# moonbow721/DPoser

Measured on AMD Instinct MI355X. Metric: poses/sec score-net train step (subVP DSM, ScoreModelFC) at global B=65536, higher is better.
Workload: dtype bf16; 1 GPU; subVP denoising-score-matching train step (fwd+bwd+clip+Adam+EMA), ScoreModelFC H=1024 E=512 2 blocks, z-scored toy-pose rows [B,63]; global_batch=65536, per_gpu_batch=65536, parallelism=dp1

## Files before the change

dposer_amd/csrc/elementwise.hip:

```cpp
#include "kernels_api.h"
#include "sde_dev.h"
#include "rng.h"

#pragma clang fp contract(off)


template <typename T> __device__ __forceinline__ void store_quad_ft(void* base, int64_t s, int c, int K, f32x4 v) {
    Quad<T>::store(reinterpret_cast<T*>(base) + FT<T>::index(s, c, K), v);
}

template <bool FAST = false>
__device__ __forceinline__ float temb_from_freq(float label, bool sin_half, float f, int fourier) {
    float arg;
    if (fourier) arg = ((logf(label) * f) * 2.0f) * 3.14159274101257324f;
    else arg = label * f;
    if (FAST && !fourier) {
        const float rev = arg * 0.15915494309189535f;
        return sin_half ? __builtin_amdgcn_sinf(rev) : __builtin_amdgcn_cosf(rev);
    }
    return sin_half ? sinf(arg) : cosf(arg);
}
template <bool FAST = false>
__device__ __forceinline__ float temb_value(float label, int e, int E, const float* freq, int fourier) {
    const int half = E >> 1;
    return temb_from_freq<FAST>(label, e < half, freq[e < half ? e : e - half], fourier);
}

template <typename Job> __device__ __forceinline__ Job kernarg_job(int index) {
    static_assert(sizeof(Job) % 4 == 0, "jobs are copied as dwords");
    typedef const uint32_t __attribute__((address_space(4))) * ConstWords;
    ConstWords w = (ConstWords)__builtin_amdgcn_kernarg_segment_ptr() + (size_t)index * (sizeof(Job) / 4);
    union { Job j; uint32_t u[sizeof(Job) / 4]; } c;
#pragma unroll
    for (unsigned i = 0; i < sizeof(Job) / 4; ++i) c.u[i] = w[i];
    return c.j;
}

template <typename T> __device__ __forceinline__ void pack_chunk(const PackJob& j, const float* flat, unsigned char* packed, int64_t chunk) {
    constexpr int EPL = FT<T>::EPL, KBS = FT<T>::KBS;
    const int kblocks = j.kpad / KBS;
    const int lane = (int)(chunk & 63);
    const int64_t blk = chunk >> 6;
    const int kb = (int)(blk % kblocks);
    const int64_t rb = blk / kblocks;
    const int r = (int)(rb * 32 + (lane & 31));
    const int k0 = kb * KBS + (lane >> 5) * EPL;
    const float* src = flat + j.src_off;
    T vals[EPL];
#pragma unroll
    for (int e = 0; e < EPL; ++e) {
        const int k = k0 + e;
        float v = 0.f;
        if (r < j.rows_valid && k < j.cols_valid) v = j.trans ? src[(int64_t)k * j.ld + r] : src[(int64_t)r * j.ld + k];
        if (sizeof(T) == 2 && j.split == 2) v = v - (float)(__bf16)v;
        vals[e] = from_f32<T>(v);
    }
    T* dst = reinterpret_cast<T*>(packed + j.dst_off) + FT<T>::index(r, j.koff + k0, j.ktot);
    *reinterpret_cast<u32x4*>(dst) = *reinterpret_cast<u32x4*>(vals);
}
__global__ void __launch_bounds__(256) k_pack(PackJobs jobs, const float* flat, unsigned char* packed) {
    (void)jobs;
    const PackJob j = kernarg_job<PackJob>((int)blockIdx.y);
    const int epl = j.f32 ? 4 : 8;
    const int64_t nchunks = (int64_t)j.rows_pad * j.kpad / epl;
    for (int64_t c = (int64_t)blockIdx.x * blockDim.x + threadIdx.x; c < nchunks; c += (int64_t)gridDim.x * blockDim.x) {
        if (j.f32) pack_chunk<float>(j, flat, packed, c);
        else pack_chunk<__bf16>(j, flat, packed, c);
    }
}
hipError_t launch_pack(const PackJobs& jobs, const float* flat, void* packed, hipStream_t st) {
    if (jobs.n <= 0) return hipSuccess;
    hipLaunchKernelGGL(k_pack, dim3(256, jobs.n), dim3(256), 0, st, jobs, flat, reinterpret_cast<unsigned char*>(packed));
    return hipGetLastError();
}

__global__ void k_bias_cat(BiasCatJobs j, const float* flat, float* dst) {
    const int i = blockIdx.x * blockDim.x + threadIdx.x;
    if (i >= j.n * j.H) return;
    const int l = i / j.H, c = i % j.H;
    int64_t a = j.a_off[0], b = j.b_off[0];
#pragma unroll
    for (int k = 1; k < 8; ++k) { a = (l == k) ? j.a_off[k] : a; b = (l == k) ? j.b_off[k] : b; }
    dst[i] = flat[a + c] + flat[b + c];
}
hipError_t launch_bias_cat(const BiasCatJobs& j, const float* flat, float* dst, hipStream_t st) {
    const int n = j.n * j.H;
    hipLaunchKernelGGL(k_bias_cat, dim3((n + 255) / 256), dim3(256), 0, st, j, flat, dst);
    return hipGetLastError();
}

template <typename T> __global__ void __launch_bounds__(256) k_prep_infer(PrepArgs a) {
    const int qx = a.Dpad >> 2, qe = a.emb ? (a.E >> 2) : 0;
    const int64_t nx = a.Bpad * qx;
    const int64_t total = nx + a.Bpad * qe;
    for (int64_t i = (int64_t)blockIdx.x * blockDim.x + threadIdx.x; i < total; i += (int64_t)gridDim.x * blockDim.x) {
        const int64_t s = i < nx ? i / qx : (i - nx) % a.Bpad;
        const int q = i < nx ? (int)(i % qx) : qx + (int)((i - nx) / a.Bpad);
        f32x4 v = {0.f, 0.f, 0.f, 0.f};
        if (q < qx) {
            const int c = q * 4;
            if (s < a.B) {
#pragma unroll
                for (int r = 0; r < 4; ++r)
                    if (c + r < a.D) v[r] = a.x[s * a.D + c + r];
            }
            store_quad_ft<T>(a.xin, s, c, a.Dpad, v);
        } else {
            const int e = (q - qx) * 4;
            const float label = s < a.B ? a.labels[s] : (a.fourier ? 1.0f : 0.0f);
#pragma unroll
            for (int r = 0; r < 4; ++r) v[r] = temb_value<sizeof(T) == 2>(label, e + r, a.E, a.freq, a.fourier);
            store_quad_ft<T>(a.emb, s, e, a.E, v);
        }
    }
}
static inline int grid_for(int64_t n, int per_block = 256, int cap = 8192) {
    int64_t g = (n + per_block - 1) / per_block;
    return (int)(g < 1 ? 1 : (g > cap ? cap : g));
}
hipError_t launch_prep_infer(const PrepArgs& a, hipStream_t st) {
    const int64_t total = a.Bpad * ((a.Dpad >> 2) + (a.emb ? (a.E >> 2) : 0));
    if (a.f32) hipLaunchKernelGGL(k_prep_infer<float>, dim3(grid_for(total)), dim3(256), 0, st, a);
    else hipLaunchKernelGGL(k_prep_infer<__bf16>, dim3(grid_for(total)), dim3(256), 0, st, a);
    return hipGetLastError();
}

struct PrepTrainDev {
    PrepTrainArgs a;
    SdeDev sde;
    float t_scale;
};
constexpr int PREP_EQ = 8;
template <typename T, bool FOURIER> __global__ void __launch_bounds__(256) k_prep_train(PrepTrainDev d) {
    const PrepTrainArgs& a = d.a;
    const int qx = a.Dpad >> 2, qe = a.E >> 2;
    const int ge = (qe + PREP_EQ - 1) / PREP_EQ;
    const int QD = (a.D + 3) >> 2;
    const int64_t nx = a.Bpad * qx;
    const int64_t total = nx + a.Bpad * ge;
    for (int64_t i = (int64_t)blockIdx.x * blockDim.x + threadIdx.x; i < total; i += (int64_t)gridDim.x * blockDim.x) {
        const int64_t s = i < nx ? i / qx : (i - nx) % a.Bpad;
        float t = a.eps;
        if (s < a.B) {
            if (a.t_in) t = a.t_in[s];
            else {
                Philox4 r = philox_at((uint64_t)s, STREAM_TRAIN_T, a.step, a.seed);
                t = u01(r.v[0]) * d.t_scale + a.eps;
            }
        }
        if (i < nx) {
            const int q = (int)(i % qx);
            f32x4 v = {0.f, 0.f, 0.f, 0.f};
            const int c = q * 4;
            f32x4 z = {0.f, 0.f, 0.f, 0.f};
            if (s < a.B && c < a.D) {
                if (a.z_in) {
#pragma unroll
                    for (int r = 0; r < 4; ++r)
                        if (c + r < a.D) z[r] = a.z_in[s * a.D + c + r];
                } else {
                    float n4[4];
                    normals4((uint64_t)s * QD + q, STREAM_TRAIN_Z, a.step, a.seed, n4);
#pragma unroll
                    for (int r = 0; r < 4; ++r)
                        if (c + r < a.D) z[r] = n4[r];
                }
                const SdeAt at = sde_at(d.sde, t);
                const float mc = at.mc, sd = at.sd;
#pragma unroll
                for (int r = 0; r < 4; ++r)
                    if (c + r < a.D) v[r] = mc * a.x0[s * a.D + c + r] + sd * z[r];
            }
            store_quad_ft<T>(a.xin, s, c, a.Dpad, v);
            *reinterpret_cast<f32x4*>(a.z_out + s * a.Dpad + c) = z;
            if (q == 0) a.t_out[s] = t;
        } else {
            const int g0 = (int)((i - nx) / a.Bpad) * PREP_EQ;
            const float label = d.sde.kind == SDE_VE ? sde_ve_sigma(d.sde.smin, d.sde.ratio, t) : t * 999.0f;
            const int half = a.E >> 1;
            f32x4 fr[PREP_EQ];
#pragma unroll
            for (int k = 0; k < PREP_EQ; ++k) {
                const int e = (g0 + k) * 4;
                fr[k] = f32x4{0.f, 0.f, 0.f, 0.f};
                if (e < a.E) fr[k] = *reinterpret_cast<const f32x4*>(a.freq + (e < half ? e : e - half));
            }
#pragma unroll
            for (int k = 0; k < PREP_EQ; ++k) {
                const int e = (g0 + k) * 4;
                if (e < a.E) {
                    f32x4 v;
#pragma unroll
                    for (int r = 0; r < 4; ++r) v[r] = temb_from_freq<sizeof(T) == 2>(label, e < half, fr[k][r], FOURIER);
                    store_quad_ft<T>(a.emb, s, e, a.E, v);
                }
            }
        }
    }
}
hipError_t launch_prep_train(const PrepTrainArgs& a, hipStream_t st) {
    PrepTrainDev d;
    d.a = a;
    d.sde = make_sde_dev(a.sde);
    d.t_scale = (float)((double)a.sde.T - (double)a.eps);
    const int64_t total = a.Bpad * ((a.Dpad >> 2) + ((a.E >> 2) + PREP_EQ - 1) / PREP_EQ);
    if (a.fourier) {
        if (a.f32) hipLaunchKernelGGL((k_prep_train<float, true>), dim3(grid_for(total)), dim3(256), 0, st, d);
        else hipLaunchKernelGGL((k_prep_train<__bf16, true>), dim3(grid_for(total)), dim3(256), 0, st, d);
    } else {
        if (a.f32) hipLaunchKernelGGL((k_prep_train<float, false>), dim3(grid_for(total)), dim3(256), 0, st, d);
        else hipLaunchKernelGGL((k_prep_train<__bf16, false>), dim3(grid_for(total)), dim3(256), 0, st, d);
    }
    return hipGetLastError();
}

__global__ void __launch_bounds__(256) k_time_embed(const float* labels, float label0, int64_t n, int64_t npad, const float* freq, int E, int fourier, float* emb) {
    const int qe = E >> 2;
    const int64_t total = npad * qe;
    for (int64_t i = (int64_t)blockIdx.x * blockDim.x + threadIdx.x; i < total; i += (int64_t)gridDim.x * blockDim.x) {
        const int64_t s = i % npad;
        const int e = (int)(i / npad) * 4;
        const float label = s < n ? (labels ? labels[s] : label0) : (fourier ? 1.0f : 0.0f);
        f32x4 v;
#pragma unroll
        for (int r = 0; r < 4; ++r) v[r] = temb_value(label, e + r, E, freq, fourier);
        store_quad_ft<float>(emb, s, e, E, v);
    }
}
__global__ void __launch_bounds__(256) k_ve_labels(float* t_inout, int n, float smin, float ratio) {
    const int i = blockIdx.x * 256 + threadIdx.x;
    if (i < n) t_inout[i] = sde_ve_sigma(smin, ratio, t_inout[i]);
}
hipError_t launch_ve_labels(float* t_inout, int n, float smin, float ratio, hipStream_t st) {
    if (n <= 0) return hipSuccess;
    hipLaunchKernelGGL(k_ve_labels, dim3((unsigned)((n + 255) / 256)), dim3(256), 0, st, t_inout, n, smin, ratio);
    return hipGetLastError();
}
hipError_t launch_time_embed(const float* labels, float label0, int64_t n, int64_t npad, const float* freq, int E, int fourier, float* emb, hipStream_t st) {
    hipLaunchKernelGGL(k_time_embed, dim3(grid_for(npad * (E >> 2))), dim3(256), 0, st, labels, label0, n, npad, freq, E, fourier, emb);
    return hipGetLastError();
}


__global__ void __launch_bounds__(256) k_out_model(OutModelArgs a) {
    const int64_t total = a.B * a.D;
    for (int64_t i = (int64_t)blockIdx.x * blockDim.x + threadIdx.x; i < total; i += (int64_t)gridDim.x * blockDim.x) {
        const int64_t s = i / a.D;
        const int c = (int)(i % a.D);
        float v = a.res[s * a.Cp + c];
        if (a.scale_by_sigma) v = v / used_sigma(a.sigmas, a.num_scales, a.labels[s], a.fourier);
        a.out[i] = v;
    }
}
hipError_t launch_out_model(const OutModelArgs& a, hipStream_t st) {
    hipLaunchKernelGGL(k_out_model, dim3(grid_for(a.B * a.D)), dim3(256), 0, st, a);
    return hipGetLastError();
}

template <typename A> struct WithSde {
    A a;
    SdeDev sde;
};
template <typename A> static hipError_t launch_quads(void (*k32)(WithSde<A>), void (*k16)(WithSde<A>), const A& a, const SdeDev& sde, hipStream_t st) {
    const WithSde<A> d = {a, sde};
    hipLaunchKernelGGL(a.f32 ? k32 : k16, dim3(grid_for(a.Bpad * (a.Dpad >> 2))), dim3(256), 0, st, d);
    return hipGetLastError();
}
template <typename A> __device__ __forceinline__ float launch_usig(const A& a, float label) {
    return a.scale_by_sigma ? used_sigma(a.sigmas, a.num_scales, label, a.scale_by_sigma == 2) : 1.0f;
}
__device__ __forceinline__ float score_of_res(const SdeDev& sde, float res, float usig, float sd_score) { return sde_score(sde, res / usig, sd_score); }
__device__ __forceinline__ float tweedie_x0(float xt, float sigma2, float score, float alpha) { return (xt + sigma2 * score) / alpha; }
__device__ __forceinline__ float snr_loss_weight(float snr) { return 0.5f * sqrtf(1.0f + snr); }
__device__ __forceinline__ float impute(float x, float m, float obs, float mc, float z, float sd) { return x * (1.0f - m) + (mc * obs + z * sd) * m; }
template <typename T> __global__ void __launch_bounds__(256) k_em_update(WithSde<EmUpdateArgs> d) {
    const EmUpdateArgs& a = d.a;
    const int qx = a.Dpad >> 2;
    const int QD = (a.D + 3) >> 2;
    const int64_t total = a.Bpad * qx;
    const float t = a.t;
    const SdeAt at = sde_at(d.sde, t);
    const float mc = at.mc, sd = at.sd, beta = at.beta, g = at.g, label = at.label;
    const float usig = launch_usig(a, label);
    float mcn = 0.f, sdn = 0.f;
    if (a.t_next >= 0.f) { const SdeAt an = sde_at(d.sde, a.t_next); mcn = an.mc; sdn = an.sd; }
    for (int64_t i = (int64_t)blockIdx.x * blockDim.x + threadIdx.x; i < total; i += (int64_t)gridDim.x * blockDim.x) {
        const int64_t s = i / qx;
        const int q = (int)(i % qx);
        const int c = q * 4;
        f32x4 xn = {0.f, 0.f, 0.f, 0.f};
        if (s < a.B && c < a.D) {
            float zp[4], zb[4], za[4];
            if (a.res && !a.pf && !a.z_pred) normals4((uint64_t)s * QD + q, STREAM_EM_NOISE, a.step, a.seed, zp);
            if (a.obs && a.res && !a.z_impB) normals4((uint64_t)s * QD + q, STREAM_IMPUTE_B, a.step, a.seed, zb);
            if (a.obs && a.t_next >= 0.f && !a.z_impA) normals4((uint64_t)s * QD + q, STREAM_IMPUTE_A, a.step + 1, a.seed, za);
#pragma unroll
            for (int r = 0; r < 4; ++r) {
                if (c + r >= a.D) continue;
                const int64_t o = s * a.D + c + r;
                float x = a.x[o];
                if (a.res) {
                    const float score = score_of_res(d.sde, a.res[s * a.Cp + c + r], usig, at.sd_score);
                    float drift = (-0.5f * beta) * x;
                    drift = drift - ((g * g) * score) * (a.pf ? 0.5f : 1.0f);
                    const float x_mean = x + drift * d.sde.dt;
                    if (a.pf) {
                        x = x_mean;
                    } else {
                        const float z = a.z_pred ? a.z_pred[o] : zp[r];
                        x = x_mean + (g * d.sde.sqrt_mdt) * z;
                    }
                    a.x_mean[o] = x_mean;
                    if (a.obs) {
                        x = impute(x, a.mask[o], a.obs[o], mc, a.z_impB ? a.z_impB[o] : zb[r], sd);
                    }
                    if (a.traj) a.traj[o] = x;
                }
                if (a.obs && a.t_next >= 0.f) {
                    x = impute(x, a.mask[o], a.obs[o], mcn, a.z_impA ? a.z_impA[o] : za[r], sdn);
                }
                a.x[o] = x;
                xn[r] = x;
            }
        }
        store_quad_ft<T>(a.xin, s, c, a.Dpad, xn);
        if (a.x_ft) store_quad_ft<float>(a.x_ft, s, c, a.Dpad, xn);
    }
}
__global__ void __launch_bounds__(256) k_ft_to_rows(const float* a_ft, float* a, const float* b_ft, float* b, int64_t B, int D, int Dpad) {
    const int qx = Dpad >> 2;
    const int64_t total = B * qx;
    for (int64_t i = (int64_t)blockIdx.x * blockDim.x + threadIdx.x; i < total; i += (int64_t)gridDim.x * blockDim.x) {
        const int64_t s = i / qx;
        const int c = (int)(i % qx) * 4;
        const int64_t off = FT<float>::index(s, c, Dpad);
        if (a_ft) {
            const f32x4 v = *reinterpret_cast<const f32x4*>(a_ft + off);
#pragma unroll
            for (int r = 0; r < 4; ++r) if (c + r < D) a[s * D + c + r] = v[r];
        }
        if (b_ft) {
            const f32x4 v = *reinterpret_cast<const f32x4*>(b_ft + off);
#pragma unroll
            for (int r = 0; r < 4; ++r) if (c + r < D) b[s * D + c + r] = v[r];
        }
    }
}
hipError_t launch_ft_to_rows(const float* a_ft, float* a, const float* b_ft, float* b, int64_t B, int64_t Bpad, int D, int Dpad, hipStream_t st) {
    (void)Bpad;
    hipLaunchKernelGGL(k_ft_to_rows, dim3(grid_for(B * (Dpad >> 2))), dim3(256), 0, st, a_ft, a, b_ft, b, B, D, Dpad);
    return hipGetLastError();
}
hipError_t launch_em_update(const EmUpdateArgs& a, hipStream_t st) { return launch_quads(k_em_update<float>, k_em_update<__bf16>, a, make_sde_dev_at(a.sde, a.t), st); }

__device__ __forceinline__ float block_sum_256(float v) {
    __shared__ float red[4];
#pragma unroll
    for (int d = 32; d >= 1; d >>= 1) v += __shfl_xor(v, d);
    const int w = threadIdx.x >> 6;
    __syncthreads();
    if ((threadIdx.x & 63) == 0) red[w] = v;
    __syncthreads();
    return red[0] + red[1] + red[2] + red[3];
}

// ... 362 lines not shown
    const AldArgs& a = d.a;
    const int qx = a.Dpad >> 2;
    const int QD = (a.D + 3) >> 2;
    const SdeAt at = sde_at(d.sde, a.t);
    const float usig = launch_usig(a, at.label);
    const float step = pc_ald_step_size(a.snr, at.sd, a.alpha);
    const float nscale = sqrtf(step * 2.0f);
    const int64_t total = a.Bpad * qx;
    for (int64_t i = (int64_t)blockIdx.x * blockDim.x + threadIdx.x; i < total; i += (int64_t)gridDim.x * blockDim.x) {
        const int64_t s = i / qx;
        const int q = (int)(i % qx);
        const int c = q * 4;
        f32x4 xn = {0.f, 0.f, 0.f, 0.f};
        if (s < a.B && c < a.D) {
            float z[4], zi[4];
            if (!a.noise) normals4((uint64_t)s * QD + q, STREAM_LANGEVIN, a.step, a.seed, z);
            if (a.obs && !a.z_imp) normals4((uint64_t)s * QD + q, STREAM_IMPUTE_A, a.imp_step, a.seed, zi);
#pragma unroll
            for (int r = 0; r < 4; ++r) {
                if (c + r >= a.D) continue;
                const int64_t o = s * a.D + c + r;
                const float g = score_of_res(d.sde, a.res[s * a.Cp + c + r], usig, at.sd_score);
                const float n = a.noise ? a.noise[o] : z[r];
                const float xm = a.x[o] + step * g;
                float x = xm + n * nscale;
                if (a.x_mean) a.x_mean[o] = xm;
                if (a.obs) {
                    x = impute(x, a.mask[o], a.obs[o], at.mc, a.z_imp ? a.z_imp[o] : zi[r], at.sd);
                }
                a.x[o] = x;
                xn[r] = x;
            }
        }
        store_quad_ft<T>(a.xin, s, c, a.Dpad, xn);
    }
}
hipError_t launch_ald_update(const AldArgs& a, hipStream_t st) { return launch_quads(k_ald_update<float>, k_ald_update<__bf16>, a, make_sde_dev_at(a.sde, a.t), st); }
struct GuidedScal { float mc, sd, sd2, beta, g, sds, usig; };
template <typename A> __device__ __forceinline__ GuidedScal guided_scalars(const A& a, const SdeDev& sde) {
    const SdeAt at = sde_at(sde, a.t);
    GuidedScal k;
    k.mc = at.mc; k.sd = at.sd; k.sd2 = at.sd * at.sd; k.beta = at.beta; k.g = at.g; k.sds = at.sd_score;
    k.usig = launch_usig(a, at.label);
    return k;
}
__device__ __forceinline__ float guided_resid(const SdeDev& sde, const GuidedScal& k, float res, float x, float obs, float m, float* score_out) {
    const float score = score_of_res(sde, res, k.usig, k.sds);
    const float y0 = tweedie_x0(x, k.sd2, score, k.mc);
    *score_out = score;
    return obs * m - y0 * m;
}
template <typename T> __global__ void __launch_bounds__(256) k_guided_resid(WithSde<GuidedArgs> d) {
    const GuidedArgs& a = d.a;
    const int qc = a.Cp >> 2;
    const int64_t total = a.Bpad * qc;
    const GuidedScal k = guided_scalars(a, d.sde);
    float acc = 0.f;
    for (int64_t i = (int64_t)blockIdx.x * blockDim.x + threadIdx.x; i < total; i += (int64_t)gridDim.x * blockDim.x) {
        const int64_t s = i / qc;
        const int c = (int)(i % qc) * 4;
        f32x4 dr = {0.f, 0.f, 0.f, 0.f};
        if (s < a.B && c < a.D) {
#pragma unroll
            for (int r = 0; r < 4; ++r) {
                if (c + r >= a.D) continue;
                const int64_t o = s * a.D + c + r;
                const float m = a.mask[o];
                float score;
                const float rr = guided_resid(d.sde, k, a.res[s * a.Cp + c + r], a.x[o], a.obs[o], m, &score);
                acc += rr * rr;
                const float gscore = ((-(m * rr)) / k.mc) * k.sd2;
                const float gmodel = d.sde.kind == SDE_VE ? gscore : -(gscore / k.sds);
                dr[r] = gmodel / k.usig;
            }
        }
        store_quad_ft<T>(a.dres, s, c, a.Cp, dr);
    }
    const float tot = block_sum_256(acc);
    if (threadIdx.x == 0) a.part[blockIdx.x] = tot;
}
hipError_t launch_guided_resid(const GuidedArgs& a, int* nblocks, hipStream_t st) {
    const WithSde<GuidedArgs> d = {a, make_sde_dev_at(a.sde, a.t)};
    const int g = grid_for(a.Bpad * (a.Cp >> 2), 256, 1024);
    *nblocks = g;
    hipLaunchKernelGGL(a.f32 ? k_guided_resid<float> : k_guided_resid<__bf16>, dim3(g), dim3(256), 0, st, d);
    return hipGetLastError();
}
template <typename T> __global__ void __launch_bounds__(256) k_guided_update(WithSde<GuidedArgs> d) {
    const GuidedArgs& a = d.a;
    const int qx = a.Dpad >> 2;
    const int QD = (a.D + 3) >> 2;
    const int64_t total = a.Bpad * qx;
    const GuidedScal k = guided_scalars(a, d.sde);
    const float norm = sqrtf(a.norm_sq[0]);
    bool bad = false;
    for (int64_t i = (int64_t)blockIdx.x * blockDim.x + threadIdx.x; i < total; i += (int64_t)gridDim.x * blockDim.x) {
        const int64_t s = i / qx;
        const int q = (int)(i % qx);
        const int c = q * 4;
        f32x4 xn = {0.f, 0.f, 0.f, 0.f};
        if (s < a.B && c < a.D) {
            float zp[4], zi[4];
            if (!a.z_pred) normals4((uint64_t)s * QD + q, STREAM_EM_NOISE, a.step, a.seed, zp);
            if (a.project && !a.z_imp) normals4((uint64_t)s * QD + q, STREAM_IMPUTE_B, a.step, a.seed, zi);
#pragma unroll
            for (int r = 0; r < 4; ++r) {
                if (c + r >= a.D) continue;
                const int64_t o = s * a.D + c + r;
                const float x0 = a.x[o], m = a.mask[o], obs = a.obs[o];
                float score;
                const float rr = guided_resid(d.sde, k, a.res[s * a.Cp + c + r], x0, obs, m, &score);
                float drift = (-0.5f * k.beta) * x0;
                drift = drift - (k.g * k.g) * score;
                const float y_mean = x0 + drift * d.sde.dt;
                const float y_hat = y_mean + (k.g * d.sde.sqrt_mdt) * (a.z_pred ? a.z_pred[o] : zp[r]);
                const float gn = (-(m * rr)) / k.mc + a.dx[o];
                const float grad = norm == 0.0f ? 0.0f : gn / norm;
                if (!isfinite(grad)) bad = true;
                float x = y_hat - a.grad_step * grad;
                a.x_mean[o] = y_mean;
                if (a.project) x = impute(x, m, obs, k.mc, a.z_imp ? a.z_imp[o] : zi[r], k.sd);
                if (a.traj) a.traj[o] = x;
                a.x[o] = x;
                xn[r] = x;
            }
        }
        store_quad_ft<T>(a.xin, s, c, a.Dpad, xn);
    }
    if (bad) atomicMin(a.nonfinite, (int32_t)a.step);
}
hipError_t launch_guided_update(const GuidedArgs& a, hipStream_t st) { return launch_quads(k_guided_update<float>, k_guided_update<__bf16>, a, make_sde_dev_at(a.sde, a.t), st); }

template <typename T> __global__ void __launch_bounds__(256) k_pack_rows(const float* x, void* xin, int64_t B, int64_t Bpad, int D, int Dpad) {
    const int qx = Dpad >> 2;
    const int64_t total = Bpad * qx;
    for (int64_t i = (int64_t)blockIdx.x * blockDim.x + threadIdx.x; i < total; i += (int64_t)gridDim.x * blockDim.x) {
        const int64_t s = i / qx;
        const int c = (int)(i % qx) * 4;
        f32x4 v = {0.f, 0.f, 0.f, 0.f};
        if (s < B)
#pragma unroll
            for (int r = 0; r < 4; ++r)
                if (c + r < D) v[r] = x[s * D + c + r];
        store_quad_ft<T>(xin, s, c, Dpad, v);
    }
}
hipError_t launch_pack_rows(const float* x, void* xin, int64_t B, int64_t Bpad, int D, int Dpad, int f32, hipStream_t st) {
    const int64_t total = Bpad * (Dpad >> 2);
    if (f32) hipLaunchKernelGGL(k_pack_rows<float>, dim3(grid_for(total)), dim3(256), 0, st, x, xin, B, Bpad, D, Dpad);
    else hipLaunchKernelGGL(k_pack_rows<__bf16>, dim3(grid_for(total)), dim3(256), 0, st, x, xin, B, Bpad, D, Dpad);
    return hipGetLastError();
}

template <typename T> __global__ void __launch_bounds__(256) k_dsm(WithSde<DsmArgs> d) {
    __shared__ float cs[256][4];
    const DsmArgs& a = d.a;
    const int qc = a.Cp >> 2;
    const int lanes = 256 / qc;
    const int q = threadIdx.x % qc, sl = threadIdx.x / qc;
    const int c = q * 4;
    float acc = 0.f;
    f32x4 csum = {0.f, 0.f, 0.f, 0.f};
    if (sl < lanes) {
        for (int64_t s = (int64_t)blockIdx.x * lanes + sl; s < a.Bpad; s += (int64_t)gridDim.x * lanes) {
            f32x4 dr = {0.f, 0.f, 0.f, 0.f};
            if (s < a.B && c < a.D) {
                const float t = a.t[s];
                const SdeAt at = sde_at(d.sde, t);
                const float sd = at.sd;
                const float usig = a.scale_by_sigma ? used_sigma(a.sigmas, a.num_scales, at.label, a.fourier) : 1.0f;
                const bool ve = d.sde.kind == SDE_VE;
#pragma unroll
                for (int r = 0; r < 4; ++r)
                    if (c + r < a.D) {
                        const float model = a.res[s * a.Cp + c + r] / usig;
                        const float score = sde_score(d.sde, model, sd);
                        const float e = score * sd + a.z[s * a.Dpad + c + r];
                        acc += e * e;
                        dr[r] = ve ? ((2.0f * e) * sd) * a.grad_scale / usig : (-2.0f * e) * a.grad_scale / usig;
                    }
            }
            store_quad_ft<T>(a.dres, s, c, a.Cp, dr);
            const f32x4 st4 = Quad<T>::round_trip(dr);
#pragma unroll
            for (int r = 0; r < 4; ++r) csum[r] += st4[r];
        }
    }
#pragma unroll
    for (int r = 0; r < 4; ++r) cs[threadIdx.x][r] = csum[r];
    const float tot = block_sum_256(acc);
    if (threadIdx.x == 0) a.loss_part[blockIdx.x] = tot * a.grad_scale;
    if (a.cs_part && threadIdx.x < qc) {
        f32x4 t4 = {0.f, 0.f, 0.f, 0.f};
        for (int l = 0; l < lanes; ++l)
#pragma unroll
            for (int r = 0; r < 4; ++r) t4[r] += cs[l * qc + threadIdx.x][r];
        *reinterpret_cast<f32x4*>(a.cs_part + (int64_t)blockIdx.x * a.Cp + c) = t4;
    }
}
hipError_t launch_dsm(const DsmArgs& a, int* nblocks, hipStream_t st) {
    const WithSde<DsmArgs> d = {a, make_sde_dev(a.sde)};
    const int lanes = 256 / (a.Cp >> 2);
    int64_t g = (a.Bpad + lanes - 1) / lanes;
    g = g < 1 ? 1 : (g > 1024 ? 1024 : g);
    *nblocks = (int)g;
    if (a.f32) hipLaunchKernelGGL(k_dsm<float>, dim3((unsigned)g), dim3(256), 0, st, d);
    else hipLaunchKernelGGL(k_dsm<__bf16>, dim3((unsigned)g), dim3(256), 0, st, d);
    return hipGetLastError();
}

template <typename T> __global__ void __launch_bounds__(256) k_silu_bwd_reduce(SiLUBwdReduceArgs a) {
    __shared__ float cs[256][4];
    constexpr bool PRECISE = sizeof(T) == 4;
    constexpr int MAXS = 8, SPT = 4;
    const int qc = a.N >> 2;
    const int lanes = 256 / qc;
    const int q = threadIdx.x % qc, sl = threadIdx.x / qc;
    const int c = q * 4;
    f32x4 csum = {0.f, 0.f, 0.f, 0.f};
    if (sl < lanes) {
        const int64_t step = (int64_t)gridDim.x * lanes;
        for (int64_t s0 = (int64_t)blockIdx.x * lanes + sl; s0 < a.Spad; s0 += step * SPT) {
            f32x4 part[SPT][MAXS], u[SPT];
#pragma unroll
            for (int i = 0; i < SPT; ++i) {
                const int64_t s = s0 + i * step;
                const bool live = s < a.B;
                const int64_t idx = live ? FT<float>::index(s, c, a.N) : 0;
#pragma unroll
                for (int k = 0; k < MAXS; ++k)
                    part[i][k] = (live && k < a.nsplit) ? Quad<float>::load(a.part + (int64_t)k * a.split_stride + idx) : f32x4{0.f, 0.f, 0.f, 0.f};
                u[i] = live ? Quad<T>::load(reinterpret_cast<const T*>(a.pre) + FT<T>::index(s, c, a.N)) : f32x4{0.f, 0.f, 0.f, 0.f};
            }
#pragma unroll
            for (int i = 0; i < SPT; ++i) {
                const int64_t s = s0 + i * step;
                if (s >= a.Spad) break;
                f32x4 acc = part[i][0];
#pragma unroll
                for (int k = 1; k < MAXS; ++k)
#pragma unroll
                    for (int r = 0; r < 4; ++r) acc[r] += part[i][k][r];
                f32x4 o = {0.f, 0.f, 0.f, 0.f};
                if (s < a.B) {
#pragma unroll
                    for (int r = 0; r < 4; ++r) o[r] = acc[r] * (a.act == DP_ACT_SWISH ? dsilu_f<PRECISE>(u[i][r]) : dact_rt<PRECISE>(u[i][r], a.act));
                }
                store_quad_ft<T>(a.out, s, c, a.N, o);
                const f32x4 st4 = Quad<T>::round_trip(o);
#pragma unroll
                for (int r = 0; r < 4; ++r) csum[r] += st4[r];
            }
        }
    }
#pragma unroll
    for (int r = 0; r < 4; ++r) cs[threadIdx.x][r] = csum[r];
    __syncthreads();
    if (threadIdx.x < qc) {
        f32x4 t4 = {0.f, 0.f, 0.f, 0.f};
        for (int l = 0; l < lanes; ++l)
#pragma unroll
            for (int r = 0; r < 4; ++r) t4[r] += cs[l * qc + threadIdx.x][r];
        *reinterpret_cast<f32x4*>(a.cs_part + (int64_t)blockIdx.x * a.N + c) = t4;
    }
}
hipError_t launch_silu_bwd_reduce(const SiLUBwdReduceArgs& a, int max_blocks, int* nblocks, hipStream_t st) {
    if (a.N % 4 != 0 || a.N > 1024) return hipErrorInvalidValue;
    if (a.nsplit < 1 || a.nsplit > 8) return hipErrorInvalidValue;
    const int lanes = 256 / (a.N >> 2);
    int64_t g = (a.Spad + lanes * 4 - 1) / (lanes * 4);
    g = g < 1 ? 1 : (g > max_blocks ? max_blocks : g);
    *nblocks = (int)g;
    if (a.f32) hipLaunchKernelGGL(k_silu_bwd_reduce<float>, dim3((unsigned)g), dim3(256), 0, st, a);
    else hipLaunchKernelGGL(k_silu_bwd_reduce<__bf16>, dim3((unsigned)g), dim3(256), 0, st, a);
    return hipGetLastError();
}

__global__ void __launch_bounds__(256) k_silu_bwd_reduce_ft(SiLUBwdReduceArgs a, __bf16* __restrict__ out_hi, __bf16* __restrict__ out_lo) {
    __shared__ float cs[256][4];
    const int kbs = a.N >> 3;
    const int kb = blockIdx.x * 4 + (threadIdx.x >> 6), lane = threadIdx.x & 63, kh = lane >> 5, r = lane & 31;
    const int c = 8 * kb + 4 * kh;
    f32x4 csum = {0.f, 0.f, 0.f, 0.f};
    const float* pre = reinterpret_cast<const float*>(a.pre);
    float* out = reinterpret_cast<float*>(a.out);
    for (int64_t rb = blockIdx.y; rb < (a.Spad >> 5); rb += gridDim.y) {
        const int64_t idx = ((rb * kbs + kb) << 8) + lane * 4;
        const bool live = rb * 32 + r < a.B;
        f32x4 acc = *reinterpret_cast<const f32x4*>(a.part + idx);
        for (int k = 1; k < a.nsplit; ++k) {
            const f32x4 v = *reinterpret_cast<const f32x4*>(a.part + (int64_t)k * a.split_stride + idx);
#pragma unroll
            for (int q = 0; q < 4; ++q) acc[q] += v[q];
        }
        const f32x4 u = *reinterpret_cast<const f32x4*>(pre + idx);
        f32x4 o = {0.f, 0.f, 0.f, 0.f};
        if (live) {
#pragma unroll
            for (int q = 0; q < 4; ++q) o[q] = acc[q] * (a.act == DP_ACT_SWISH ? dsilu_f<true>(u[q]) : dact_rt<true>(u[q], a.act));
        }
        *reinterpret_cast<f32x4*>(out + idx) = o;
        if (out_hi) {
            __bf16 h4[4], l4[4];
#pragma unroll
            for (int q = 0; q < 4; ++q) { h4[q] = (__bf16)o[q]; l4[q] = (__bf16)(o[q] - (float)h4[q]); }
            const int64_t pidx = (((rb * (a.N >> 4) + (kb >> 1)) << 6) + ((kb & 1) << 5) + r) * 8 + kh * 4;
            *reinterpret_cast<uint2*>(out_hi + pidx) = *reinterpret_cast<const uint2*>(h4);
            *reinterpret_cast<uint2*>(out_lo + pidx) = *reinterpret_cast<const uint2*>(l4);
        }
#pragma unroll
        for (int q = 0; q < 4; ++q) csum[q] += o[q];
    }
#pragma unroll
    for (int q = 0; q < 4; ++q) cs[threadIdx.x][q] = csum[q];
    __syncthreads();
    if (r == 0) {
        f32x4 t4 = {0.f, 0.f, 0.f, 0.f};
        for (int l = 0; l < 32; ++l)
#pragma unroll
            for (int q = 0; q < 4; ++q) t4[q] += cs[threadIdx.x + l][q];
        *reinterpret_cast<f32x4*>(a.cs_part + (int64_t)blockIdx.y * a.N + c) = t4;
    }
}
hipError_t launch_silu_bwd_reduce_ft(const SiLUBwdReduceArgs& a, void* out_hi, void* out_lo, int max_blocks, int* nblocks, hipStream_t st) {
    if (a.N % 32 != 0 || !a.f32 || a.nsplit < 1) return hipErrorInvalidValue;
    int64_t gy = a.Spad >> 5;
    gy = gy > 256 ? 256 : gy;
    gy = gy > max_blocks ? max_blocks : gy;
    *nblocks = (int)gy;
    hipLaunchKernelGGL(k_silu_bwd_reduce_ft, dim3((unsigned)(a.N / 32), (unsigned)gy), dim3(256), 0, st, a, (__bf16*)out_hi, (__bf16*)out_lo);
    return hipGetLastError();
}

template <typename T> __global__ void __launch_bounds__(256) k_dres_from_dout(DresArgs a) {
    const int qc = a.Cp >> 2;
    const int64_t total = a.Bpad * qc;
    for (int64_t i = (int64_t)blockIdx.x * blockDim.x + threadIdx.x; i < total; i += (int64_t)gridDim.x * blockDim.x) {
        const int64_t s = i / qc;
// ... 662 lines not shown
```

Measured before the change: 20.98 million poses/s.

## Restructure train prep and DSM kernels around row blocks with LDS staging

The train prep kernel now handles 32-row blocks per workgroup. It computes t, mc, sd and label once per row into LDS, caches the frequency table in LDS, stages the perturbed input in LDS, and writes it and the time embedding with 16-byte coalesced stores in the fragment-tiled layout. For small batches it uses 1024-thread blocks. The DSM loss kernel precomputes per-row sigma terms into shared memory once per tile and batches vectorised loads of residual and noise four iterations at a time to raise memory-level parallelism. The new code adds divisibility requirements (Bpad%32, Dpad%64, E%128) and extra barriers, and the LDS footprint depends on Dpad.

```diff
diff --git a/dposer_amd/csrc/elementwise.hip b/dposer_amd/csrc/elementwise.hip
--- a/dposer_amd/csrc/elementwise.hip
+++ b/dposer_amd/csrc/elementwise.hip
@@ -130,72 +130,101 @@
     SdeDev sde;
     float t_scale;
 };
-constexpr int PREP_EQ = 8;
-template <typename T, bool FOURIER> __global__ void __launch_bounds__(256) k_prep_train(PrepTrainDev d) {
+template <typename T, bool FOURIER, int NT> __global__ void __launch_bounds__(NT) k_prep_train(PrepTrainDev d) {
+    extern __shared__ __attribute__((aligned(16))) unsigned char prep_lds[];
+    constexpr int EPL = FT<T>::EPL, KBS = FT<T>::KBS;
     const PrepTrainArgs& a = d.a;
-    const int qx = a.Dpad >> 2, qe = a.E >> 2;
-    const int ge = (qe + PREP_EQ - 1) / PREP_EQ;
-    const int QD = (a.D + 3) >> 2;
-    const int64_t nx = a.Bpad * qx;
-    const int64_t total = nx + a.Bpad * ge;
-    for (int64_t i = (int64_t)blockIdx.x * blockDim.x + threadIdx.x; i < total; i += (int64_t)gridDim.x * blockDim.x) {
-        const int64_t s = i < nx ? i / qx : (i - nx) % a.Bpad;
-        float t = a.eps;
-        if (s < a.B) {
-            if (a.t_in) t = a.t_in[s];
-            else {
-                Philox4 r = philox_at((uint64_t)s, STREAM_TRAIN_T, a.step, a.seed);
-                t = u01(r.v[0]) * d.t_scale + a.eps;
-            }
-        }
-        if (i < nx) {
-            const int q = (int)(i % qx);
-            f32x4 v = {0.f, 0.f, 0.f, 0.f};
-            const int c = q * 4;
-            f32x4 z = {0.f, 0.f, 0.f, 0.f};
-            if (s < a.B && c < a.D) {
-                if (a.z_in) {
-#pragma unroll
-                    for (int r = 0; r < 4; ++r)
-                        if (c + r < a.D) z[r] = a.z_in[s * a.D + c + r];
-                } else {
-                    float n4[4];
-                    normals4((uint64_t)s * QD + q, STREAM_TRAIN_Z, a.step, a.seed, n4);
-#pragma unroll
-                    for (int r = 0; r < 4; ++r)
-                        if (c + r < a.D) z[r] = n4[r];
+    const int qx = a.Dpad >> 2, QD = (a.D + 3) >> 2, half = a.E >> 1;
+    float* s_freq = reinterpret_cast<float*>(prep_lds);
+    float* s_mc = s_freq + half;
+    float* s_sd = s_mc + 32;
+    float* s_label = s_sd + 32;
+    T* s_x = reinterpret_cast<T*>(s_label + 32);
+    const int tid = threadIdx.x;
+    for (int i = tid; i < half; i += NT) s_freq[i] = a.freq[i];
+    const int nq = 32 * qx;
+    const int nch_x = 32 * a.Dpad / EPL, nch_e = 32 * a.E / EPL;
+    const int64_t nrb = a.Bpad >> 5;
+    auto draw = [&](int64_t s0, int k, f32x4& z, f32x4& x0) {
+        const int r = k / qx, q = k - r * qx, c = q * 4;
+        const int64_t s = s0 + r;
+        z = f32x4{0.f, 0.f, 0.f, 0.f};
+        x0 = z;
+        if (s < a.B && c < a.D) {
+            if (a.z_in) {
+#pragma unroll
+                for (int e = 0; e < 4; ++e)
+                    if (c + e < a.D) z[e] = a.z_in[s * a.D + c + e];
+            } else {
+                float n4[4];
+                normals4((uint64_t)s * QD + q, STREAM_TRAIN_Z, a.step, a.seed, n4);
+#pragma unroll
+                for (int e = 0; e < 4; ++e)
+                    if (c + e < a.D) z[e] = n4[e];
+            }
+#pragma unroll
+            for (int e = 0; e < 4; ++e)
+                if (c + e < a.D) x0[e] = a.x0[s * a.D + c + e];
+        }
+    };
+    auto perturb = [&](int64_t s0, int k, const f32x4& z, const f32x4& x0) {
+        const int r = k / qx, q = k - r * qx, c = q * 4;
+        const int64_t s = s0 + r;
+        f32x4 v = {0.f, 0.f, 0.f, 0.f};
+        if (s < a.B && c < a.D) {
+            const float mc = s_mc[r], sd = s_sd[r];
+#pragma unroll
+            for (int e = 0; e < 4; ++e)
+                if (c + e < a.D) v[e] = mc * x0[e] + sd * z[e];
+        }
+        Quad<T>::store(s_x + FT<T>::index(r, c, a.Dpad), v);
+        *reinterpret_cast<f32x4*>(a.z_out + s * a.Dpad + c) = z;
+    };
+    for (int64_t rb = blockIdx.x; rb < nrb; rb += gridDim.x) {
+        const int64_t s0 = rb << 5;
+        if (tid < 32) {
+            const int64_t s = s0 + tid;
+            float t = a.eps, mc = 0.f, sd = 0.f;
+            if (s < a.B) {
+                if (a.t_in) t = a.t_in[s];
+                else {
+                    Philox4 r = philox_at((uint64_t)s, STREAM_TRAIN_T, a.step, a.seed);
+                    t = u01(r.v[0]) * d.t_scale + a.eps;
                 }
                 const SdeAt at = sde_at(d.sde, t);
-                const float mc = at.mc, sd = at.sd;
-#pragma unroll
-                for (int r = 0; r < 4; ++r)
-                    if (c + r < a.D) v[r] = mc * a.x0[s * a.D + c + r] + sd * z[r];
-            }
-            store_quad_ft<T>(a.xin, s, c, a.Dpad, v);
-            *reinterpret_cast<f32x4*>(a.z_out + s * a.Dpad + c) = z;
-            if (q == 0) a.t_out[s] = t;
-        } else {
-            const int g0 = (int)((i - nx) / a.Bpad) * PREP_EQ;
-            const float label = d.sde.kind == SDE_VE ? sde_ve_sigma(d.sde.smin, d.sde.ratio, t) : t * 999.0f;
-            const int half = a.E >> 1;
-            f32x4 fr[PREP_EQ];
-#pragma unroll
-            for (int k = 0; k < PREP_EQ; ++k) {
-                const int e = (g0 + k) * 4;
-                fr[k] = f32x4{0.f, 0.f, 0.f, 0.f};
-                if (e < a.E) fr[k] = *reinterpret_cast<const f32x4*>(a.freq + (e < half ? e : e - half));
-            }
-#pragma unroll
-            for (int k = 0; k < PREP_EQ; ++k) {
-                const int e = (g0 + k) * 4;
-                if (e < a.E) {
-                    f32x4 v;
-#pragma unroll
-                    for (int r = 0; r < 4; ++r) v[r] = temb_from_freq<sizeof(T) == 2>(label, e < half, fr[k][r], FOURIER);
-                    store_quad_ft<T>(a.emb, s, e, a.E, v);
-                }
-            }
-        }
+                mc = at.mc; sd = at.sd;
+            }
+            a.t_out[s] = t;
+            s_mc[tid] = mc; s_sd[tid] = sd;
+            s_label[tid] = d.sde.kind == SDE_VE ? sde_ve_sigma(d.sde.smin, d.sde.ratio, t) : t * 999.0f;
+        }
+        f32x4 za, xa, zb, xb;
+        const bool qa = NT <= 256 || tid < nq, qb = NT <= 256 || tid + NT < nq;
+        if (qa) draw(s0, tid, za, xa);
+        if (qb) draw(s0, tid + NT, zb, xb);
+        __syncthreads();
+        if (qa) perturb(s0, tid, za, xa);
+        if (qb) perturb(s0, tid + NT, zb, xb);
+        for (int k = tid + 2 * NT; k < nq; k += NT) {
+            draw(s0, k, za, xa);
+            perturb(s0, k, za, xa);
+        }
+        T* embp = reinterpret_cast<T*>(a.emb) + rb * 32 * a.E;
+        for (int ch = tid; ch < nch_e; ch += NT) {
+            const int r = ch & 31, e0 = (ch >> 6) * KBS + ((ch >> 5) & 1) * EPL;
+            const float label = s_label[r];
+            const bool sin_half = e0 < half;
+            const float* f = s_freq + (sin_half ? e0 : e0 - half);
+            T vals[EPL];
+#pragma unroll
+            for (int e = 0; e < EPL; ++e) vals[e] = from_f32<T>(temb_from_freq<sizeof(T) == 2>(label, sin_half, f[e], FOURIER));
+            *reinterpret_cast<u32x4*>(embp + (int64_t)ch * EPL) = *reinterpret_cast<u32x4*>(vals);
+        }
+        __syncthreads();
+        T* xinp = reinterpret_cast<T*>(a.xin) + rb * 32 * a.Dpad;
+        for (int ch = tid; ch < nch_x; ch += NT)
+            *reinterpret_cast<u32x4*>(xinp + (int64_t)ch * EPL) = *reinterpret_cast<const u32x4*>(s_x + ch * EPL);
+        __syncthreads();
     }
 }
 hipError_t launch_prep_train(const PrepTrainArgs& a, hipStream_t st) {
@@ -203,14 +232,19 @@
     d.a = a;
     d.sde = make_sde_dev(a.sde);
     d.t_scale = (float)((double)a.sde.T - (double)a.eps);
-    const int64_t total = a.Bpad * ((a.Dpad >> 2) + ((a.E >> 2) + PREP_EQ - 1) / PREP_EQ);
+    const int grid = grid_for(a.Bpad >> 5, 1, 8192);
+    const size_t lds = (size_t)(a.E >> 1) * 4 + 3 * 32 * 4 + (size_t)32 * a.Dpad * (a.f32 ? 4 : 2);
+    if (lds > 64 * 1024 || (a.Bpad & 31) || (a.Dpad & 63) || (a.E & 127)) return hipErrorInvalidValue;
+    void (*k)(PrepTrainDev);
+    const bool wide = (a.Bpad >> 5) <= 256;
     if (a.fourier) {
-        if (a.f32) hipLaunchKernelGGL((k_prep_train<float, true>), dim3(grid_for(total)), dim3(256), 0, st, d);
-        else hipLaunchKernelGGL((k_prep_train<__bf16, true>), dim3(grid_for(total)), dim3(256), 0, st, d);
+        if (a.f32) k = wide ? k_prep_train<float, true, 1024> : k_prep_train<float, true, 256>;
+        else k = wide ? k_prep_train<__bf16, true, 1024> : k_prep_train<__bf16, true, 256>;
     } else {
-        if (a.f32) hipLaunchKernelGGL((k_prep_train<float, false>), dim3(grid_for(total)), dim3(256), 0, st, d);
-        else hipLaunchKernelGGL((k_prep_train<__bf16, false>), dim3(grid_for(total)), dim3(256), 0, st, d);
-    }
+        if (a.f32) k = wide ? k_prep_train<float, false, 1024> : k_prep_train<float, false, 256>;
+        else k = wide ? k_prep_train<__bf16, false, 1024> : k_prep_train<__bf16, false, 256>;
+    }
+    hipLaunchKernelGGL(k, dim3(grid), dim3(wide ? 1024 : 256), lds, st, d);
     return hipGetLastError();
 }
 
@@ -879,38 +913,75 @@
     return hipGetLastError();
 }
 
+constexpr int DSM_U = 4;
 template <typename T> __global__ void __launch_bounds__(256) k_dsm(WithSde<DsmArgs> d) {
     __shared__ float cs[256][4];
+    __shared__ float s_sd[256], s_usig[256];
     const DsmArgs& a = d.a;
     const int qc = a.Cp >> 2;
     const int lanes = 256 / qc;
     const int q = threadIdx.x % qc, sl = threadIdx.x / qc;
     const int c = q * 4;
+    const int trips = 256 / lanes;
+    const int64_t stride = (int64_t)gridDim.x * lanes;
+    const bool ve = d.sde.kind == SDE_VE;
     float acc = 0.f;
     f32x4 csum = {0.f, 0.f, 0.f, 0.f};
-    if (sl < lanes) {
-        for (int64_t s = (int64_t)blockIdx.x * lanes + sl; s < a.Bpad; s += (int64_t)gridDim.x * lanes) {
-            f32x4 dr = {0.f, 0.f, 0.f, 0.f};
-            if (s < a.B && c < a.D) {
-                const float t = a.t[s];
-                const SdeAt at = sde_at(d.sde, t);
-                const float sd = at.sd;
-                const float usig = a.scale_by_sigma ? used_sigma(a.sigmas, a.num_scales, at.label, a.fourier) : 1.0f;
-                const bool ve = d.sde.kind == SDE_VE;
-#pragma unroll
-                for (int r = 0; r < 4; ++r)
-                    if (c + r < a.D) {
-                        const float model = a.res[s * a.Cp + c + r] / usig;
-                        const float score = sde_score(d.sde, model, sd);
-                        const float e = score * sd + a.z[s * a.Dpad + c + r];
-                        acc += e * e;
-                        dr[r] = ve ? ((2.0f * e) * sd) * a.grad_scale / usig : (-2.0f * e) * a.grad_scale / usig;
+    f32x4 R[DSM_U], Z[DSM_U];
+    auto fetch = [&](int64_t base, int it0) {
+#pragma unroll
+        for (int u = 0; u < DSM_U; ++u) {
+            const int64_t s = base + (int64_t)(it0 + u) * stride + sl;
+            R[u] = f32x4{0.f, 0.f, 0.f, 0.f};
+            Z[u] = R[u];
+            if (sl < lanes && it0 + u < trips && s < a.B && c < a.D) {
+                R[u] = *reinterpret_cast<const f32x4*>(a.res + s * a.Cp + c);
+                Z[u] = *reinterpret_cast<const f32x4*>(a.z + s * a.Dpad + c);
+            }
+        }
+    };
+    for (int64_t base = (int64_t)blockIdx.x * lanes; base < a.Bpad; base += stride * trips) {
+        fetch(base, 0);
+        __syncthreads();
+        {
+            const int it = threadIdx.x / lanes, l = threadIdx.x - it * lanes;
+            const int64_t s = base + (int64_t)it * stride + l;
+            float sd = 0.f, usig = 1.0f;
+            if (it < trips && s < a.B) {
+                const SdeAt at = sde_at(d.sde, a.t[s]);
+                sd = at.sd;
+                usig = a.scale_by_sigma ? used_sigma(a.sigmas, a.num_scales, at.label, a.fourier) : 1.0f;
+            }
+            s_sd[threadIdx.x] = sd; s_usig[threadIdx.x] = usig;
+        }
+        __syncthreads();
+        if (sl < lanes) {
+            for (int it0 = 0; it0 < trips && base + (int64_t)it0 * stride < a.Bpad; it0 += DSM_U) {
+                if (it0) fetch(base, it0);
+#pragma unroll
+                for (int u = 0; u < DSM_U; ++u) {
+                    const int it = it0 + u;
+                    const int64_t s = base + (int64_t)it * stride + sl;
+                    if (it >= trips || s >= a.Bpad) break;
+                    f32x4 dr = {0.f, 0.f, 0.f, 0.f};
+                    if (s < a.B && c < a.D) {
+                        const float sd = s_sd[it * lanes + sl], usig = s_usig[it * lanes + sl];
+#pragma unroll
+                        for (int r = 0; r < 4; ++r)
+                            if (c + r < a.D) {
+                                const float model = R[u][r] / usig;
+                                const float score = sde_score(d.sde, model, sd);
+                                const float e = score * sd + Z[u][r];
+                                acc += e * e;
+                                dr[r] = ve ? ((2.0f * e) * sd) * a.grad_scale / usig : (-2.0f * e) * a.grad_scale / usig;
+                            }
                     }
-            }
-            store_quad_ft<T>(a.dres, s, c, a.Cp, dr);
-            const f32x4 st4 = Quad<T>::round_trip(dr);
-#pragma unroll
-            for (int r = 0; r < 4; ++r) csum[r] += st4[r];
+                    store_quad_ft<T>(a.dres, s, c, a.Cp, dr);
+                    const f32x4 st4 = Quad<T>::round_trip(dr);
+#pragma unroll
+                    for (int r = 0; r < 4; ++r) csum[r] += st4[r];
+                }
+            }
         }
     }
 #pragma unroll
```

New measurement: 20.95 million poses/s. Within noise of the previous version (-0.2%).
